# marl/l3embedding

Hardware: AMD Instinct MI355X
Metric: AVC training pairs/sec (1s audio + 224x224 frame) (higher is better)
Workload: dtype f32; 1 GPU; full cnn_L3_melspec2 AVC training step (audio+vision+fusion, fwd+bwd+Adam), batch 64 per GPU, global batch 64, fp32, inputs resident in HBM; global_batch=64, parallelism=dp1, fp32_conv=f4x4

## Files before the change

l3embedding_amd/csrc/conv_wino.hip:

```cpp
#include "kernels.h"
#include "device_common.h"
#include "wino_common.h"

#include <stdlib.h>

#include <atomic>
#include <mutex>

namespace l3 {

bool conv_wino4_selected(const ConvGeom& g);
double conv_wino4_executed_flops(const ConvGeom& g);
int conv_wino4_blocks(const ConvGeom& g, int n);
void conv_wino4_transform_weights(const float* w, float* u, const ConvGeom& g, bool from_fwd_for_dgrad, hipStream_t s);
void conv_wino4_launch(const float* x, const float* u, const float* bias, float* y, const ConvGeom& g, int n, hipStream_t s,
                       float* stat_part, int stat_mode, const BnBwdFuse* bn_bwd);

#ifdef L3_EXPERIMENTS
bool conv_wino_bx6_ok(const ConvGeom& g);
int conv_wino_bx6_blocks(const ConvGeom& g, int n);
double conv_wino_bx6_executed_flops(const ConvGeom& g);
void conv_wino_bx6_transform_weights(const float* w, float* u, const ConvGeom& g, bool from_fwd_for_dgrad, hipStream_t s);
void conv_wino_bx6_launch(const float* x, const float* u, const float* bias, float* y, const ConvGeom& g, int n, hipStream_t s,
                          float* stat_part, int stat_mode, const BnBwdFuse* bn_bwd);
#else
static inline bool conv_wino_bx6_ok(const ConvGeom&) { return false; }
static inline int conv_wino_bx6_blocks(const ConvGeom&, int) { return 0; }
static inline double conv_wino_bx6_executed_flops(const ConvGeom&) { return 0.0; }
static inline void conv_wino_bx6_transform_weights(const float*, float*, const ConvGeom&, bool, hipStream_t) {}
static inline void conv_wino_bx6_launch(const float*, const float*, const float*, float*, const ConvGeom&, int, hipStream_t, float*, int,
                                        const BnBwdFuse*) {}
#endif

namespace {

// ... 153 lines not shown
            if (c + 1 < a.nchunks) issue(0, c + 1);
            compute(1, FalseT{});
            stage_barrier();
            if (c + 1 < a.nchunks) {
                if (c + 2 < a.nchunks) issue(1, c + 2);
                compute(0, FalseT{});
                stage_barrier();
            }
        }
    };
    issue(0, 0);
    __syncthreads();
    if (xi == 1) {
        if (nu == 1) stage_loop(TrueT{}, TrueT{}); else stage_loop(TrueT{}, FalseT{});
    } else {
        if (nu == 1) stage_loop(FalseT{}, TrueT{}); else stage_loop(FalseT{}, FalseT{});
    }

    wino_output<BTX, SM, 16>(a, acc1, smem, t, wave, lane, R0, tx0, n0, mb);
    if (dyn && t == 0) {
        int nx = wq_base(0, xcd) + 8 * claim_k;
        if (nx >= total_tiles) nx = wq_claim(a.work, xcd, 1, 0, total_tiles);
        Qw[(it + 1) & 1] = nx;
    }
    }
    if (dyn && t == 0) wq_leave(a.work, (int)gridDim.x);
}

__global__ __launch_bounds__(256) void wino_weights_kernel(const float* __restrict__ w, float* __restrict__ u, int Cin,
                                                           int Cout, int dgrad) {
    const int idx = blockIdx.x * 256 + threadIdx.x;
    if (idx >= Cin * Cout) return;
    const int k = idx % Cout, c = idx / Cout;
    float g[3][3];
#pragma unroll
    for (int kh = 0; kh < 3; ++kh)
#pragma unroll
        for (int kw = 0; kw < 3; ++kw)
            g[kh][kw] = dgrad ? w[((size_t)((2 - kh) * 3 + (2 - kw)) * Cout + k) * Cin + c]
                              : w[((size_t)(kh * 3 + kw) * Cin + c) * Cout + k];
    float gg[4][3];
#pragma unroll
    for (int kw = 0; kw < 3; ++kw) {
        gg[0][kw] = g[0][kw];
        gg[1][kw] = 0.5f * (g[0][kw] + g[1][kw] + g[2][kw]);
        gg[2][kw] = 0.5f * (g[0][kw] - g[1][kw] + g[2][kw]);
        gg[3][kw] = g[2][kw];
    }
#pragma unroll
    for (int xi = 0; xi < 4; ++xi) {
        const float o0 = gg[xi][0];
        const float o1 = 0.5f * (gg[xi][0] + gg[xi][1] + gg[xi][2]);
        const float o2 = 0.5f * (gg[xi][0] - gg[xi][1] + gg[xi][2]);
        const float o3 = gg[xi][2];
        const float o[4] = {o0, o1, o2, o3};
#pragma unroll
        for (int nu = 0; nu < 4; ++nu)
            u[(((size_t)(xi * 4 + nu) * (Cin >> 2) + (c >> 2)) * Cout + k) * 4 + (c & 3)] = o[nu];
    }
}

template <int BTX, int SM>
void launch_wino2(const WinoArgs& a, hipStream_t s) {
    using G = WinoGeom<BTX>;
    static std::once_flag once[L3_MAX_DEVICES];
    int dev = 0;
    (void)hipGetDevice(&dev);
    std::call_once(once[dev & (L3_MAX_DEVICES - 1)], [] {
        (void)hipFuncSetAttribute((const void*)conv_wino_kernel<BTX, SM>, hipFuncAttributeMaxDynamicSharedMemorySize, (int)G::LDS_BYTES + 16);
    });
    static const int persist_env = l3_knob("L3_WINO_PERSIST") ? atoi(l3_knob("L3_WINO_PERSIST")) : -1;
    const int persist = persist_env >= 0 ? persist_env : 1;
    static int cus[L3_MAX_DEVICES] = {0};
    int& ncu = cus[dev & (L3_MAX_DEVICES - 1)];
    if (ncu == 0) {
        hipDeviceProp_t prop;
        ncu = hipGetDeviceProperties(&prop, dev) == hipSuccess && prop.multiProcessorCount >= 8 ? prop.multiProcessorCount / 8 * 8 : 256;
    }
    const int total = a.mblocks * a.nblocks;
    const int ncu_k = l3_knob("L3_W4_NCU") ? atoi(l3_knob("L3_W4_NCU")) / 8 * 8 : 0;
    const int ncu_eff = ncu_k > 0 && ncu_k < ncu ? ncu_k : ncu;
    const int dyn_on = l3_knob("L3_W4_DYNAMIC") ? atoi(l3_knob("L3_W4_DYNAMIC")) : a.dynamic;
    WinoArgs m = a;
    m.work = persist && total > ncu_eff && dyn_on ? persistent_work_counters(s) : nullptr;
    hipLaunchKernelGGL((conv_wino_kernel<BTX, SM>), dim3(persist && total > ncu_eff ? ncu_eff : total), dim3(1024), G::LDS_BYTES + 16, s, m);
}
template <int BTX>
void launch_wino(const WinoArgs& a, hipStream_t s) {
    if (a.stat_part != nullptr && a.bb.x != nullptr)
        launch_wino2<BTX, 2>(a, s);
    else if (a.stat_part != nullptr)
// ... 25 lines not shown
    return p;
}

}

bool conv_wino_ok(const ConvGeom& g) {
    static const int enabled = l3_knob("L3_WINOGRAD") ? atoi(l3_knob("L3_WINOGRAD")) : 1;
    return enabled && g.KH == 3 && g.KW == 3 && g.padT == 1 && g.padL == 1 && g.Ho == g.H && g.Wo == g.W &&
           g.Cin % 8 == 0 && g.Cout % 64 == 0 && (size_t)16 * g.Cin * g.Cout * 4 < (1ull << 31) &&
           (size_t)g.H * g.W * (g.Cin > g.Cout ? g.Cin : g.Cout) * 4 < (1ull << 31);
}

static int wino_chunk_samples(const ConvGeom& g) {
    const size_t per_sample = (size_t)g.H * g.W * (g.Cin > g.Cout ? g.Cin : g.Cout) * 4;
    size_t nc = ((1ull << 31) - 1) / per_sample;
    const size_t row_cap = ((1u << 22) - 1) / (size_t)((g.H + 1) / 2);
    if (nc > row_cap) nc = row_cap;
    if (nc > (size_t)g.N) nc = (size_t)g.N;
    return nc < 1 ? 1 : (int)nc;
}

static bool use_bx6(const ConvGeom& g) { return g.f2x2 == 2 && conv_wino_ok(g) && conv_wino_bx6_ok(g); }
static bool use_wino4(const ConvGeom& g) { return !use_bx6(g) && conv_wino_ok(g) && conv_wino4_selected(g); }

bool conv_wino_is_bx6(const ConvGeom& g) { return use_bx6(g); }

double conv_wino_executed_flops(const ConvGeom& g) {
    if (use_bx6(g)) return conv_wino_bx6_executed_flops(g);
    if (use_wino4(g)) return conv_wino4_executed_flops(g);
    return 2.0 * 16.0 * (double)g.N * ((g.H + 1) / 2) * ((g.W + 1) / 2) * (double)g.Cin * (double)g.Cout;
}

size_t conv_wino_floats(const ConvGeom& g) { return conv_wino_ok(g) ? (size_t)36 * g.Cin * g.Cout : 0; }

void conv_wino_transform_weights(const float* w, float* u, const ConvGeom& g, bool from_fwd_for_dgrad, hipStream_t s) {
    if (use_bx6(g)) return conv_wino_bx6_transform_weights(w, u, g, from_fwd_for_dgrad, s);
    if (use_wino4(g)) return conv_wino4_transform_weights(w, u, g, from_fwd_for_dgrad, s);
    const int total = g.Cin * g.Cout;
    hipLaunchKernelGGL(wino_weights_kernel, dim3((total + 255) / 256), dim3(256), 0, s, w, u, g.Cin, g.Cout,
                       from_fwd_for_dgrad ? 1 : 0);
}

static int stat_blocks_of(const ConvGeom& g, int algo) {
    const int nc = wino_chunk_samples(g);
    int blocks = 0;
    for (int n0 = 0; n0 < g.N; n0 += nc) {
        ConvGeom gc = g;
        gc.N = g.N - n0 < nc ? g.N - n0 : nc;
        blocks += algo == 1 ? conv_wino4_blocks(g, gc.N) : algo == 2 ? conv_wino_bx6_blocks(g, gc.N) : wino_plan(gc).mblocks;
    }
    return blocks;
}

int conv_wino_stat_blocks(const ConvGeom& g) { return conv_wino_ok(g) ? stat_blocks_of(g, use_bx6(g) ? 2 : use_wino4(g) ? 1 : 0) : 0; }

int conv_wino_stat_blocks_max(const ConvGeom& g) {
    if (!conv_wino_ok(g)) return 0;
    int m = stat_blocks_of(g, 0);
    const int b = stat_blocks_of(g, 1);
    if (b > m) m = b;
    if (g.Cin % 16 == 0 && conv_wino_bx6_ok(g)) {
        const int c = stat_blocks_of(g, 2);
        if (c > m) m = c;
    }
    return m;
}
// ... 69 lines not shown
```

l3embedding_amd/csrc/conv_wino4.hip:

```cpp
#include "kernels.h"
#include "device_common.h"

#include <stdlib.h>
#include <string.h>

#include <mutex>
#include <vector>

namespace l3 {

namespace {

struct Wino4Args {
    const float* x;
    const float* u;
    const float* bias;
    float* y;
    int N, H, W, Cin, Cout;
    int TY, TX;
    int tiles;
    int mblocks, nblocks, nchunks;
    float inv_tpi, inv_tx;
    float* stat_part;
    int stat_mode;
    BnBwdFuse bb;
    int stagger_cycles, stagger_groups;
    int lt_first, lt_end, ksplit;
    int* work;
    float* ypart;
    int solo;
    int dynamic;
    float* tail_buf;
    size_t tail_cap;
};
// ... 566 lines not shown
                        red[((jn * 2 + which) * NS + slot) * 32 + o_c32] = stv[jn][which];
                    }
                }
        }
        lds_barrier();
        if (t < 128) {
            const int c32 = t & 31, which = (t >> 5) & 1, jn = t >> 6;
            float sum = 0.f;
#pragma unroll
            for (int r = 0; r < NS; ++r) sum += red[((jn * 2 + which) * NS + r) * 32 + c32];
            a.stat_part[((size_t)mb * 2 + which) * a.Cout + n0 + jn * 32 + c32] = sum;
        }
    }
    if (!worker) __builtin_amdgcn_s_waitcnt(0x0070 | (0xF << 8));
    if (dyn && wave == 11 && lane0 == 0) {
        asm volatile("" ::: "memory");
        int nx = -1;
        if (has_next) {
            nx = wq_base(a.lt_first, xcd) + 8 * claim_k;
            if (nx >= a.lt_end) nx = wq_claim(a.work, xcd, 1, a.lt_first, a.lt_end);
        }
        Qw[it & 1] = nx;
    }
    have0 = has_next;
    }
    if (dyn && t == 0) wq_leave(a.work, (int)gridDim.x);
}

__global__ __launch_bounds__(256) void wino4_weights_kernel(const float* __restrict__ w, float* __restrict__ u, int Cin,
                                                            int Cout, int dgrad) {
    const int idx = blockIdx.x * 256 + threadIdx.x;
    if (idx >= Cin * Cout) return;
    const int k = idx % Cout, c = idx / Cout;
    float g[3][3];
#pragma unroll
    for (int kh = 0; kh < 3; ++kh)
#pragma unroll
        for (int kw = 0; kw < 3; ++kw)
            g[kh][kw] = dgrad ? w[((size_t)((2 - kh) * 3 + (2 - kw)) * Cout + k) * Cin + c]
                              : w[((size_t)(kh * 3 + kw) * Cin + c) * Cout + k];
    auto gmul = [](float a0, float a1, float a2, float* o) {
        const float s02 = a0 + a2;
        o[0] = a0;
        o[1] = (-1.f / 3.f) * (s02 + a1);
        o[2] = (1.f / 3.f) * (s02 - a1);
        o[3] = (1.f / 15.f) * fmaf(2.f, a1, fmaf(4.f, a2, a0));
        o[4] = (-4.f / 15.f) * fmaf(-2.f, a1, fmaf(4.f, a0, a2));
        o[5] = a2;
    };
    float gg[6][3];
#pragma unroll
    for (int kw = 0; kw < 3; ++kw) {
        float o[6];
        gmul(g[0][kw], g[1][kw], g[2][kw], o);
#pragma unroll
        for (int xi = 0; xi < 6; ++xi) gg[xi][kw] = o[xi];
    }
    const int c8 = c >> 3, hf = (c >> 2) & 1, sub = (c >> 1) & 1, c2 = c & 1;
#pragma unroll
    for (int xi = 0; xi < 6; ++xi) {
        float o[6];
        gmul(gg[xi][0], gg[xi][1], gg[xi][2], o);
#pragma unroll
        for (int nu = 0; nu < 6; ++nu)
            u[(((((size_t)(xi * 6 + nu) * (Cin >> 3) + c8) * 2 + sub) * 2 + hf) * Cout + k) * 2 + c2] = o[nu];
    }
}

template <int SM>
__global__ __launch_bounds__(256) void wino4_tail_reduce_kernel(Wino4Args a) {
    __shared__ float red[2][64][16];
    const int t = threadIdx.x, q = t & 3, slot = t >> 2;
    const int blk = (int)blockIdx.x >> 2, cg = (int)blockIdx.x & 3;
    const int lt = a.lt_first + blk;
    const int logical = xcd_remap(lt, a.mblocks * a.nblocks);
    const int nb = logical % a.nblocks, mb = logical / a.nblocks;
    const int n0 = nb * 64, T0 = mb * W4_TILES;
    const int cl = cg * 16 + 4 * q;
    const int ch = n0 + cl;
    f32x4 bz = {0.f, 0.f, 0.f, 0.f};
    if (a.bias != nullptr) bz = *reinterpret_cast<const f32x4*>(a.bias + ch);
    f32x4 bsc = bz, bsh = bz, bmu = bz, brs = bz;
    if constexpr (SM == 2) {
        bsc = *reinterpret_cast<const f32x4*>(a.bb.scale + ch);
        bsh = *reinterpret_cast<const f32x4*>(a.bb.shift + ch);
        bmu = *reinterpret_cast<const f32x4*>(a.bb.mean + ch);
        const f32x4 var = *reinterpret_cast<const f32x4*>(a.bb.var + ch);
#pragma unroll
        for (int c = 0; c < 4; ++c) brs[c] = rsqrtf(var[c] + a.bb.eps);
    }
    const bool srelu = SM == 1 && a.stat_mode == 2;
    float st0[4] = {0.f, 0.f, 0.f, 0.f}, st1[4] = {0.f, 0.f, 0.f, 0.f};
    const float* part = a.ypart + (size_t)blk * a.ksplit * (W4_TILES * 16 * 64) + cl;
    for (int it = 0; it < 8; ++it) {
        const int tp = it * 64 + slot, tl = tp >> 4, px = tp & 15;
        const int T = T0 + tl;
        f32x4 sum = {0.f, 0.f, 0.f, 0.f};
#pragma unroll 4
        for (int sl = 0; sl < a.ksplit; ++sl) sum += *reinterpret_cast<const f32x4*>(part + ((size_t)sl * W4_TILES * 16 + tp) * 64);
// ... 233 lines not shown
```

l3embedding_amd/csrc/engine.hip:

```cpp
#include <hip/hip_runtime.h>
#include "knobs.h"

#include <cmath>
#include <cstdio>
#include <cstdlib>
#include <cstring>
#include <map>
#include <string>
#include <vector>

#include "../../include/l3hip.h"
#include "comm.h"
#include "kernels.h"

namespace {

using namespace l3;

static thread_local std::string g_create_error;

constexpr float BN_EPS = 1e-3f;
constexpr float BN_MOMENTUM = 0.99f;
constexpr float L2_WEIGHT = 1e-5f;
constexpr float ADAM_B1 = 0.9f, ADAM_B2 = 0.999f, ADAM_EPS = 1e-8f;
// ... 8 lines not shown
    float* g = nullptr;
    int N = 0, H = 0, W = 0, C = 0;
    int64_t batch_stride = 0;
    bool alias = false;
    bool d_bf16 = false, g_bf16 = false;
    int64_t numel() const { return (int64_t)N * H * W * C; }
    int64_t rows() const { return (int64_t)N * H * W; }
};

struct Param {
    std::string name;
    int ndim = 0;
    int64_t shape[4] = {1, 1, 1, 1};
    bool trainable = false;
    int kind = 0;
    int64_t numel = 0;
    int bucket = 0;
    float* d = nullptr;
    float* g = nullptr;
};

struct Op {
    OpKind kind;
    std::string name;
    int in = 0, out = 0;
    int block = 0, bucket = 0;
    int kh = 0, kw = 0, cout = 0;
    bool same = false;
    ConvGeom geom{};
    ConvGeom dgeom{};
    int p_kernel = -1, p_bias = -1;
    float* wflip = nullptr;
    float *wino_uf = nullptr, *wino_ud = nullptr;
    int in_bn = -1;
    bool fused_first = false;
    bool defer_apply = false;
    int bn_defer = -1;
    const float* apply_coeffs = nullptr;
    float *xaug = nullptr, *gaug = nullptr;
    ConvGeom ageom{};
    int bn_follow = -1;
    int stats_nblk = 0;
    bool need_dx = true;
    int dy_to_bn = -1;
    float* xwin = nullptr;
    int bwd_part_blocks = 0;
    int p_gamma = -1, p_beta = -1, p_mmean = -1, p_mvar = -1;
    bool fused_relu = false;
    bool prerelu = false;
    int fuse_pool = -1;
    int bias_param = -1;
    bool fused_into_bn = false;
    bool bias_by_bn = false;
    float *mean = nullptr, *var = nullptr, *scale = nullptr, *shift = nullptr;
    float *biased_mean = nullptr, *biased_var = nullptr;
    PoolGeom pg{};
};

struct Tower {
    std::string prefix;
    std::vector<Tensor> t;
    std::vector<Op> ops;
    int nblocks = 0;
    int emb_conv_op = -1;
};

// ... 992 lines not shown
        }
    } else if (f.folded) {
        float* fe = e->frames;
        float* fo = e->frames + (size_t)M * f.ke;
        {
            ProfScope ps(e, F_FRONTEND, 0.0);
            frame_audio_folded(e->audio, fe, fo, B, AUDIO_T, f, e->stream);
        }
        ProfScope ps(e, F_FRONTEND, 2.0 * M * (double)f.n_dft * 2.0 * f.n_freq, nullptr,
                     2.0 * M * (double)(f.ke + f.ko) * f.nc);
        const ConvGeom ge{1, 1, M, f.ke, 1, M, f.nc, 1, 1, 0, 0}, go{1, 1, M, f.ko, 1, M, f.nc, 1, 1, 0, 0};
        conv_fwd(fe, e->wdft, nullptr, e->spec, ge, e->stream);
        conv_fwd(fo, e->wdft + (size_t)f.ke * f.nc, nullptr, e->spec + (size_t)M * f.nc, go, e->stream);
    } else {
        {
            ProfScope ps(e, F_FRONTEND, 0.0);
            frame_audio(e->audio, e->frames, B, AUDIO_T, f, e->stream);
        }
        ConvGeom g{1, 1, M, f.n_dft, 1, M, f.ncols_pad, 1, 1, 0, 0};
        ProfScope ps(e, F_FRONTEND, 2.0 * M * (double)f.n_dft * 2.0 * f.n_freq);
        conv_fwd(e->frames, e->wdft, nullptr, e->spec, g, e->stream);
    }
    {
        ProfScope ps(e, F_FRONTEND, f.n_mels ? 2.0 * B * f.n_frames * (double)f.n_freq * f.n_mels : 0.0);
        spec_to_features(e->spec, e->melw, e->mel_start, e->mel_len, e->mel_off, e->aud.t[0].d, B, f, e->stream, e->dft_nyq);
        if (f.db) db_normalize(e->aud.t[0].d, e->smax, B, e->aud.t[0].batch_stride, e->cfg.db_max_scope, e->stream);
    }
    return L3_OK;
}

static inline double act_bytes(const Tensor& t) { return (double)t.numel() * (t.d_bf16 ? 2.0 : 4.0); }
static inline double grad_bytes(const Tensor& t) { return (double)t.numel() * (t.g_bf16 ? 2.0 : 4.0); }

void tower_forward(l3_engine* e, Tower& tw, bool training) {
    for (auto& op : tw.ops) {
        Tensor& x = tw.t[op.in];
        Tensor& y = tw.t[op.out];
        switch (op.kind) {
            case OP_CONV: {
                const bool mp = e->cfg.dtype == L3_DTYPE_BF16 && conv_bf16_ok(op.geom);
                ProfScope ps(e, F_CONV_FWD, conv_flops(op.geom), op.name.c_str(),
                             op.wino_uf && !mp ? conv_wino_executed_flops(op.geom) : -1.0);
                ps.bytes(act_bytes(x) + act_bytes(y) + (double)e->params[op.p_kernel].numel * 4.0);
                static const int epi_stats = l3_knob("L3_EPILOGUE_STATS") ? atoi(l3_knob("L3_EPILOGUE_STATS")) : 1;
                if (op.wino_uf && !mp)
                    conv_wino_transform_weights(e->params[op.p_kernel].d, op.wino_uf, op.geom, false, e->stream);
                if (mp) {
                    if (x.d_bf16)
                        conv_weights_bf16(e->params[op.p_kernel].d, op.wflip, op.kh, op.kw, x.C, op.cout, true, e->stream);
                    else
                        conv_flip_weights(e->params[op.p_kernel].d, op.wflip, op.kh, op.kw, x.C, op.cout, e->stream);
                    const bool mstats = epi_stats && training && x.d_bf16 && op.bn_follow >= 0 && e->stat_scratch != nullptr;
                    conv_bf16_fwd(x.d, op.wflip, e->params[op.p_bias].d, y.d, op.geom, e->stream, x.d_bf16,
                                  mstats ? e->stat_scratch : nullptr, mstats ? (tw.ops[op.bn_follow].prerelu ? 2 : 1) : 0,
                                  y.d_bf16);
                    if (op.bn_follow >= 0) tw.ops[op.bn_follow].stats_nblk = mstats ? conv_bf16_stat_blocks(op.geom) : 0;
                    break;
                }
                if (conv_first_ok(op.geom)) {
                    const bool fstats = epi_stats && training && op.bn_follow >= 0 && e->stat_scratch != nullptr;
                    conv_first_fwd(x.d, e->params[op.p_kernel].d, e->params[op.p_bias].d, y.d, op.geom, e->stream,
                                   fstats ? e->stat_scratch : nullptr, fstats ? (tw.ops[op.bn_follow].prerelu ? 2 : 1) : 0,
                                   y.d_bf16);
                    if (op.bn_follow >= 0) tw.ops[op.bn_follow].stats_nblk = fstats ? conv_first_stat_blocks(op.geom) : 0;
                    break;
                }
                const bool stats = epi_stats && training && op.wino_uf && op.bn_follow >= 0 && e->stat_scratch != nullptr &&
                                   conv_wino_stat_blocks(op.geom) > 0;
                conv_fwd(x.d, e->params[op.p_kernel].d, e->params[op.p_bias].d, y.d, op.geom, e->stream, op.wino_uf,
                         stats ? e->stat_scratch : nullptr, stats ? (tw.ops[op.bn_follow].prerelu ? 2 : 1) : 0);
                if (op.bn_follow >= 0) tw.ops[op.bn_follow].stats_nblk = stats ? conv_wino_stat_blocks(op.geom) : 0;
                break;
            }
            case OP_BN: {
                ProfScope ps(e, F_ELEMWISE, 0.0);
                {
                    double by = !training ? 0.0 : op.stats_nblk > 0 ? (double)op.stats_nblk * 2 * x.C * 4 : act_bytes(x);
                    if (training && op.fused_first) by += act_bytes(x) + (double)x.rows() * (&op + 1)->ageom.Cin * 4.0;
                    if (op.fuse_pool >= 0) {
// ... 150 lines not shown
                    ProfScope ps(e, F_ELEMWISE, 0.0);
                    ps.bytes(grad_bytes(y));
                    colsum(y.g, e->params[op.p_bias].g, e->red_scratch, y.rows(), y.C, e->stream);
                }
                if (op.need_dx) {
                    ProfScope ps(e, F_CONV_DGRAD, conv_flops(op.geom), op.name.c_str(),
                                 op.wino_ud && !(e->cfg.dtype == L3_DTYPE_BF16 && conv_bf16_ok(op.dgeom))
                                     ? conv_wino_executed_flops(op.dgeom)
                                     : -1.0);
                    ps.bytes(grad_bytes(y) + grad_bytes(x) + (double)e->params[op.p_kernel].numel * 4.0);
                    if (!conv_dgrad_small(y.g, e->params[op.p_kernel].d, x.g, op.geom, e->stream)) {
                        if (e->cfg.dtype == L3_DTYPE_BF16 && conv_bf16_ok(op.dgeom)) {
                            if (y.g_bf16) {
                                conv_weights_bf16(e->params[op.p_kernel].d, op.wflip, op.kh, op.kw, x.C, op.cout, false,
                                                  e->stream);
                                Op* bn = training && op.dy_to_bn >= 0 && e->stat_scratch != nullptr && x.g_bf16 &&
                                                 conv_bf16_halo_ok(op.dgeom) && tw.t[tw.ops[op.dy_to_bn].in].d_bf16
                                             ? &tw.ops[op.dy_to_bn]
                                             : nullptr;
                                if (bn != nullptr && bn->fuse_pool >= 0 && (bn->xwin == nullptr || x.batch_stride != (int64_t)x.H * x.W * x.C))
                                    bn = nullptr;
                                if (bn != nullptr) {
                                    const BnBwdFuse bb{bn->fuse_pool >= 0 ? bn->xwin : tw.t[bn->in].d, bn->scale, bn->shift, bn->mean, bn->var,
                                                       BN_EPS, bn->fused_relu ? 1 : 0};
                                    conv_bf16_fwd(y.g, op.wflip, nullptr, x.g, op.dgeom, e->stream, true, e->stat_scratch, 0, true, &bb);
                                    bn->bwd_part_blocks = conv_bf16_stat_blocks(op.dgeom);
                                } else {
                                    conv_bf16_fwd(y.g, op.wflip, nullptr, x.g, op.dgeom, e->stream, true, nullptr, 0, x.g_bf16);
                                }
                            } else {
                                conv_bf16_fwd(y.g, e->params[op.p_kernel].d, nullptr, x.g, op.dgeom, e->stream);
                            }
                        } else if (op.wino_ud) {
                            conv_wino_transform_weights(e->params[op.p_kernel].d, op.wino_ud, op.dgeom, true, e->stream);
                            Op* bn = training && op.dy_to_bn >= 0 && e->stat_scratch != nullptr && !x.g_bf16 ? &tw.ops[op.dy_to_bn] : nullptr;
                            if (bn != nullptr && bn->fuse_pool >= 0 && (bn->xwin == nullptr || x.batch_stride != (int64_t)x.H * x.W * x.C))
                                bn = nullptr;
                            if (bn != nullptr && !tw.t[bn->in].d_bf16 && conv_wino_ok(op.dgeom)) {
                                const BnBwdFuse bb{bn->fuse_pool >= 0 ? bn->xwin : tw.t[bn->in].d, bn->scale, bn->shift, bn->mean, bn->var,
                                                   BN_EPS, bn->fused_relu ? 1 : 0};
                                conv_fwd(y.g, nullptr, nullptr, x.g, op.dgeom, e->stream, op.wino_ud, e->stat_scratch, 0, &bb);
                                bn->bwd_part_blocks = conv_wino_stat_blocks(op.dgeom);
                            } else {
                                conv_fwd(y.g, nullptr, nullptr, x.g, op.dgeom, e->stream, op.wino_ud);
                            }
                        } else {
                            conv_flip_weights(e->params[op.p_kernel].d, op.wflip, op.kh, op.kw, x.C, op.cout, e->stream);
                            conv_fwd(y.g, op.wflip, nullptr, x.g, op.dgeom, e->stream);
                        }
                    }
                }
                break;
            }
            default: break;
        }
    }
}

void set_solo(l3_engine* e, Tower& tw, int v) {
    for (auto& op : tw.ops)
        if (op.kind == OP_CONV) {
            op.geom.solo = op.dgeom.solo = v;
            op.geom.dynamic = op.dgeom.dynamic = e->comm != nullptr ? 1 : 0;
            float* ts = v ? e->w4_tail : nullptr;
            op.geom.tail_scratch = op.dgeom.tail_scratch = ts;
            op.geom.tail_scratch_bytes = op.dgeom.tail_scratch_bytes = ts ? conv_wino4_tail_scratch_bytes() : 0;
        }
}

void l2_sums(l3_engine* e) {
    SumsqSegs segs{};
    int nl2 = 0;
    for (auto& s : e->segments) nl2 += s.l2 ? 1 : 0;
    if (nl2 <= SUMSQ_MAX_SEGS) {
        for (auto& s : e->segments)
            if (s.l2) {
                segs.off[segs.count] = s.off;
                segs.n[segs.count++] = s.n;
            }
        sumsq_multi(e->arena_p, segs, e->l2part, e->sq_scratch, e->stream);
        return;
    }
    int si = 0;
    for (auto& s : e->segments)
        if (s.l2) sumsq(e->arena_p + s.off, s.n, e->l2part + si++, e->sq_scratch, e->stream);
}

int forward_all(l3_engine* e, bool training) {
    int rc;
    set_solo(e, e->vis, 0);
    set_solo(e, e->aud, 0);
    if (e->side && e->overlap) {
        HIPCHK(e, hipEventRecord(e->ev_fork, e->stream));
        HIPCHK(e, hipStreamWaitEvent(e->side, e->ev_fork, 0));
        l2_sums(e);
        {
            SideScope sd(e);
            if ((rc = run_frontend(e))) return rc;
            tower_forward(e, e->aud, training);
            HIPCHK(e, hipEventRecord(e->ev_join, e->stream));
        }
        tower_forward(e, e->vis, training);
        HIPCHK(e, hipStreamWaitEvent(e->stream, e->ev_join, 0));
    } else {
        l2_sums(e);
        if ((rc = run_frontend(e))) return rc;
        tower_forward(e, e->vis, training);
        tower_forward(e, e->aud, training);
    }
    ProfScope ps(e, F_HEAD, 0.0);
    const int D = e->nv + e->na;
    dense_fwd(e->h0, e->params[e->p_w1].d, e->params[e->p_b1].d, e->h1, e->B, D, e->head, 1, e->stream);
    dense_fwd(e->h1, e->params[e->p_w2].d, e->params[e->p_b2].d, e->logits, e->B, e->head, 2, 0, e->stream);
    e->last_training = training;
    return L3_OK;
}

void loss_and_head_backward(l3_engine* e, bool backward) {
    ProfScope ps(e, F_HEAD, 0.0);
    const int gb = e->cfg.global_batch > 0 ? e->cfg.global_batch : e->B;
    softmax_ce(e->logits, e->labels, e->probs, e->dlogits, e->stats, e->B, 1.0f / (float)gb, e->stream);
    if (!backward) return;
    const int D = e->nv + e->na;
    dense_bwd_w(e->h1, e->dlogits, e->params[e->p_w2].g, e->params[e->p_b2].g, e->B, e->head, 2, e->stream);
// ... 53 lines not shown
    e->bn_table = dev;
    return L3_OK;
}

int bn_stats_pack(l3_engine* e, int world) {
    int rc = ensure_bn_table(e);
    if (rc) return rc;
    if (e->bn_pack_floats == 0) return L3_OK;
    if (e->bn_send == nullptr && (rc = dev_alloc_t(e, &e->bn_send, (size_t)e->bn_pack_floats))) return rc;
    if (e->bn_gathered_world < world) {
        if ((rc = dev_alloc_t(e, &e->bn_gathered, (size_t)e->bn_pack_floats * world))) return rc;
        e->bn_gathered_world = world;
    }
    bn_moving_pack(e->bn_table, e->bn_table_n, e->bn_table_max_c, e->bn_send, e->stream);
    return L3_OK;
}

int do_update(l3_engine* e, float lr, float grad_scale) {
    {
        ProfScope ps(e, F_ADAM, 0.0);
        e->adam_t += 1;
        const double t = (double)e->adam_t;
        const float lr_t = lr * (sqrtf(1.f - powf(ADAM_B2, (float)t)) / (1.f - powf(ADAM_B1, (float)t)));
        for (size_t i = 0; i < e->segments.size(); ++i) {
            const auto& s = e->segments[i];
            int64_t n = s.n;
            const int64_t n_l2 = s.l2 ? s.n : 0;
            if (s.l2 && i + 1 < e->segments.size() && !e->segments[i + 1].l2 && e->segments[i + 1].off == s.off + s.n)
                n += e->segments[++i].n;
            adam_step(e->arena_p + s.off, e->arena_g + s.off, e->arena_m + s.off, e->arena_v + s.off, n, n_l2, 2.f * L2_WEIGHT,
                      lr_t, ADAM_B1, ADAM_B2, ADAM_EPS, grad_scale, e->stream);
        }
    }
    ProfScope ps(e, F_ELEMWISE, 0.0);
    int rc = ensure_bn_table(e);
    if (rc) return rc;
    const int replicas = e->bn_replicas_armed;
    e->bn_replicas_armed = 0;
    e->bn_step += replicas > 0 ? replicas : 1;
    bn_moving_update_all(e->bn_table, e->bn_table_n, e->bn_table_max_c, BN_MOMENTUM, e->cfg.bn_zero_debias, e->bn_step, e->stream,
                         replicas > 0 ? e->bn_gathered : nullptr, replicas, e->bn_pack_floats);
    return L3_OK;
}

int read_results(l3_engine* e, float* loss, float* acc, float* probs, float* logits) {
    HIPCHK(e, l3::stream_wait(e->stream));
    prof_collect(e);
    float st[16], l2[64];
    HIPCHK(e, hipMemcpy(st, e->stats, sizeof(st), hipMemcpyDeviceToHost));
    HIPCHK(e, hipMemcpy(l2, e->l2part, sizeof(l2), hipMemcpyDeviceToHost));
    double reg = 0.0;
    int si = 0;
    for (auto& s : e->segments)
        if (s.l2) reg += (double)L2_WEIGHT * (double)l2[si++];
    if (loss) *loss = (float)((double)st[0] / (double)e->B + reg);
    if (acc) *acc = st[1] / (float)e->B;
    if (probs) HIPCHK(e, hipMemcpy(probs, e->probs, (size_t)e->B * 2 * 4, hipMemcpyDeviceToHost));
    if (logits) HIPCHK(e, hipMemcpy(logits, e->logits, (size_t)e->B * 2 * 4, hipMemcpyDeviceToHost));
    return L3_OK;
}

int upload_inputs(l3_engine* e, const float* video, const float* audio, const float* labels) {
    const int B = e->B;
    e->staged = false;
    e->gains_valid = false;
    if (video) HIPCHK(e, hipMemcpyAsync(e->video, video, (size_t)B * 224 * 224 * 3 * 4, hipMemcpyHostToDevice, e->stream));
// ... 190 lines not shown
    if (ndim) *ndim = p.ndim;
    if (shape)
        for (int i = 0; i < 4; ++i) shape[i] = i < p.ndim ? p.shape[i] : 1;
    if (trainable) *trainable = p.trainable ? 1 : 0;
    if (numel) *numel = p.numel;
    return L3_OK;
}

static int find_param(l3_engine* e, const char* name, int64_t numel, Param** out) {
    if (!e || !name) return L3_EINVAL;
    auto it = e->pindex.find(name);
    if (it == e->pindex.end()) {
        e->err = std::string("unknown parameter: ") + name;
        return L3_EINVAL;
    }
    Param& p = e->params[it->second];
    if (p.numel != numel) {
        e->err = std::string("size mismatch for ") + name + ": expected " + std::to_string(p.numel) + " got " +
                 std::to_string(numel);
        return L3_EINVAL;
    }
    *out = &p;
    return L3_OK;
}

int l3_set_param(l3_engine* e, const char* name, const float* src, int64_t numel) {
    Param* p;
    int rc = find_param(e, name, numel, &p);
    if (rc) return rc;
    HIPCHK(e, hipSetDevice(e->cfg.device));
    HIPCHK(e, l3::stream_wait(e->stream));
    HIPCHK(e, hipMemcpy(p->d, src, (size_t)numel * 4, hipMemcpyHostToDevice));
    if (p->kind == PK_CONST) e->consts_dirty = true;
    return L3_OK;
}

int l3_get_param(l3_engine* e, const char* name, float* dst, int64_t numel) {
    Param* p;
    int rc = find_param(e, name, numel, &p);
    if (rc) return rc;
    HIPCHK(e, hipSetDevice(e->cfg.device));
    HIPCHK(e, l3::stream_wait(e->stream));
    HIPCHK(e, hipMemcpy(dst, p->d, (size_t)numel * 4, hipMemcpyDeviceToHost));
    return L3_OK;
}

int l3_get_grad(l3_engine* e, const char* name, float* dst, int64_t numel) {
    Param* p;
    int rc = find_param(e, name, numel, &p);
    if (rc) return rc;
    if (!p->trainable) {
        e->err = std::string("not trainable: ") + name;
        return L3_EINVAL;
    }
    HIPCHK(e, hipSetDevice(e->cfg.device));
    HIPCHK(e, l3::stream_wait(e->stream));
    HIPCHK(e, hipMemcpy(dst, p->g, (size_t)numel * 4, hipMemcpyDeviceToHost));
    return L3_OK;
}

int l3_reset_optimizer(l3_engine* e) {
    if (!e) return L3_EINVAL;
    HIPCHK(e, hipSetDevice(e->cfg.device));
    HIPCHK(e, hipMemsetAsync(e->arena_m, 0, (size_t)e->n_train * 4, e->stream));
    HIPCHK(e, hipMemsetAsync(e->arena_v, 0, (size_t)e->n_train * 4, e->stream));
    e->adam_t = 0;
// ... 13 lines not shown
    if (!dst || !src) return L3_EINVAL;
    if (dst == src) return L3_OK;
    if (dst->cfg.model_type != src->cfg.model_type || dst->params.size() != src->params.size() ||
        dst->n_train != src->n_train || dst->cfg.device != src->cfg.device) {
        dst->err = "l3_copy_state: engines differ in model type or device";
        return L3_EINVAL;
    }
    HIPCHK(dst, hipSetDevice(dst->cfg.device));
    HIPCHK(dst, l3::stream_wait(src->stream));
    if (src->side) HIPCHK(dst, l3::stream_wait(src->side));
    const size_t nb = (size_t)src->n_train * 4;
    HIPCHK(dst, hipMemcpyAsync(dst->arena_p, src->arena_p, nb, hipMemcpyDeviceToDevice, dst->stream));
    HIPCHK(dst, hipMemcpyAsync(dst->arena_m, src->arena_m, nb, hipMemcpyDeviceToDevice, dst->stream));
    HIPCHK(dst, hipMemcpyAsync(dst->arena_v, src->arena_v, nb, hipMemcpyDeviceToDevice, dst->stream));
    for (size_t i = 0; i < src->params.size(); ++i) {
        const Param& ps = src->params[i];
        if (ps.trainable) continue;
        HIPCHK(dst, hipMemcpyAsync(dst->params[i].d, ps.d, (size_t)ps.numel * 4, hipMemcpyDeviceToDevice, dst->stream));
    }
    Tower* dt[2] = {&dst->vis, &dst->aud};
    Tower* st[2] = {&src->vis, &src->aud};
    for (int t = 0; t < 2; ++t)
        for (size_t i = 0; i < st[t]->ops.size(); ++i) {
            const Op& so = st[t]->ops[i];
            Op& dop = dt[t]->ops[i];
            if (so.kind != OP_BN) continue;
            const size_t n = (size_t)(st[t]->t[so.in].C + 3) / 4 * 4 * 4;
            HIPCHK(dst, hipMemcpyAsync(dop.biased_mean, so.biased_mean, n, hipMemcpyDeviceToDevice, dst->stream));
            HIPCHK(dst, hipMemcpyAsync(dop.biased_var, so.biased_var, n, hipMemcpyDeviceToDevice, dst->stream));
        }
    dst->adam_t = src->adam_t;
    dst->bn_step = src->bn_step;
    dst->consts_dirty = true;
    HIPCHK(dst, l3::stream_wait(dst->stream));
    return L3_OK;
}

int l3_optimizer_steps(const l3_engine* e, int64_t* adam_t, int64_t* bn_steps) {
    if (!e) return L3_EINVAL;
    if (adam_t) *adam_t = e->adam_t;
    if (bn_steps) *bn_steps = e->bn_step;
    return L3_OK;
}

int l3_upload_batch(l3_engine* e, const float* video, const float* audio, const float* labels) {
    if (!e) return L3_EINVAL;
    HIPCHK(e, hipSetDevice(e->cfg.device));
    return upload_inputs(e, video, audio, labels);
}

int l3_upload_batch_raw(l3_engine* e, const uint8_t* video_u8, const int16_t* audio_i16, const int32_t* labels_i32) {
    if (!e) return L3_EINVAL;
    HIPCHK(e, hipSetDevice(e->cfg.device));
    const int B = e->B;
    e->staged = false;
    e->gains_valid = false;
    if (video_u8) {
        HIPCHK(e, hipMemcpyAsync(e->raw_video, video_u8, (size_t)B * 224 * 224 * 3, hipMemcpyHostToDevice, e->stream));
        preprocess_video(e->raw_video, e->video, (int64_t)B * 224 * 224 * 3, e->stream);
    }
    if (audio_i16) {
        HIPCHK(e, hipMemcpyAsync(e->raw_audio, audio_i16, (size_t)B * AUDIO_T * 2, hipMemcpyHostToDevice, e->stream));
        preprocess_audio(e->raw_audio, e->audio, (int64_t)B * AUDIO_T, e->stream);
    }
    if (labels_i32) {
        HIPCHK(e, hipMemcpyAsync(e->raw_labels, labels_i32, (size_t)B * 2 * 4, hipMemcpyHostToDevice, e->stream));
// ... 122 lines not shown
    HIPCHK(e, l3::stream_wait(e->stream));
    HIPCHK(e, hipMemcpy(gains, e->aug_gains, (size_t)e->B * sizeof(double), hipMemcpyDeviceToHost));
    return L3_OK;
}

int l3_step_forward(l3_engine* e, int training) {
    if (!e) return L3_EINVAL;
    HIPCHK(e, hipSetDevice(e->cfg.device));
    e->bucket_ready = -1;
    e->bn_replicas_armed = 0;
    e->bn_packed = false;
    if (training) {
        const int slot = (int)(e->steps_enqueued & 1);
        if (e->ev_step_set[slot]) HIPCHK(e, l3::event_wait(e->ev_step[slot]));
    }
    int rc = adopt_staged(e);
    if (rc) return rc;
    rc = forward_all(e, training != 0);
    if (rc) return rc;
    loss_and_head_backward(e, training != 0);
    e->fwd_done = true;
    HIPCHK(e, hipGetLastError());
    return L3_OK;
}

int l3_tower_step(l3_engine* e, int tower, int backward) {
    if (!e || (tower != 0 && tower != 1)) return L3_EINVAL;
    HIPCHK(e, hipSetDevice(e->cfg.device));
    int rc = adopt_staged(e);
    if (rc) return rc;
    Tower& tw = tower == 0 ? e->vis : e->aud;
    if (tower == 1 && (rc = run_frontend(e))) return rc;
    set_solo(e, tw, 1);
    tower_forward(e, tw, true);
    if (backward) {
        const int width = tower == 0 ? e->nv : e->na;
        fill(e->dh0, 1.0f / ((float)e->B * (float)width), (int64_t)e->B * (e->nv + e->na), e->stream);
        for (int b = tw.nblocks - 1; b >= 0; --b) tower_backward_block(e, tw, b, true);
    }
    e->fwd_done = false;
    HIPCHK(e, hipGetLastError());
    return L3_OK;
}

int l3_step_bucket_count(const l3_engine* e) { return e ? (int)e->buckets.size() : L3_EINVAL; }

int l3_step_backward_bucket(l3_engine* e, int bucket) {
    if (!e) return L3_EINVAL;
    if (!e->fwd_done) {
        e->err = "l3_step_backward_bucket before l3_step_forward";
        return L3_ESTATE;
    }
    if (!e->last_training && e->cfg.dtype == L3_DTYPE_BF16) {
        e->err = "inference-mode gradients are available in L3_DTYPE_F32 engines only";
        return L3_ESTATE;
    }
    HIPCHK(e, hipSetDevice(e->cfg.device));
    int rc = backward_bucket(e, bucket);
    if (rc) return rc;
    HIPCHK(e, hipGetLastError());
    return L3_OK;
}

int l3_step_update(l3_engine* e, float lr, float grad_scale) {
    if (!e) return L3_EINVAL;
    if (!e->fwd_done || !e->last_training) {
// ... 429 lines not shown
}

static int embed_rows(l3_engine* e, bool vision, const EmbedSource& src, int64_t n, int ph, int pw, int64_t D, float* out) {
    Tower& tw = vision ? e->vis : e->aud;
    const int B = e->B;
    int64_t cap_rows = (int64_t)(EMBED_OUT_BYTES / ((size_t)D * 4)) / B * B;
    if (cap_rows < B) cap_rows = B;
    const int64_t need_rows = (n + B - 1) / B * B;
    if (cap_rows > need_rows) cap_rows = need_rows;
    int rc = dev_grow_t(e, &e->emb_out, &e->emb_out_cap, (size_t)cap_rows * D);
    if (rc) return rc;
    const Tensor& t = tw.t[tw.ops[tw.emb_conv_op].out];
    PoolGeom pg{};
    pg.N = B; pg.H = t.H; pg.W = t.W; pg.C = t.C; pg.ph = ph; pg.pw = pw; pg.sh = ph; pg.sw = pw;
    tf_same(t.H, ph, ph, &pg.Ho, &pg.padT);
    tf_same(t.W, pw, pw, &pg.Wo, &pg.padL);
    pg.out_batch_stride = D;
    const size_t per = vision ? (size_t)224 * 224 * 3 : (size_t)AUDIO_T;
    float* dst_in = vision ? e->video : e->audio;
    int64_t f0 = 0;
    for (int64_t s0 = 0; s0 < n; s0 += B) {
        const int64_t cnt = n - s0 < B ? n - s0 : B;
        if (src.host) {
            HIPCHK(e, hipMemcpyAsync(dst_in, src.host + (size_t)s0 * per, (size_t)cnt * per * 4, hipMemcpyHostToDevice, e->stream));
            if (cnt < B) HIPCHK(e, hipMemsetAsync(dst_in + (size_t)cnt * per, 0, (size_t)(B - cnt) * per * 4, e->stream));
        } else {
            gather_frames(src.samples, src.table + 3 * s0, dst_in, B, (int)cnt, AUDIO_T, e->stream);
        }
        if (!vision) {
            rc = run_frontend(e);
            if (rc) return rc;
        }
        set_solo(e, tw, 1);
        tower_forward(e, tw, false);
        maxpool_fwd(t.d, e->emb_out + (size_t)(s0 - f0) * D, pg, e->stream);
        if (s0 + cnt == n || s0 + 2 * B - f0 > cap_rows) {
            HIPCHK(e, hipMemcpyAsync(out + (size_t)f0 * D, e->emb_out, (size_t)(s0 + cnt - f0) * D * 4, hipMemcpyDeviceToHost, e->stream));
            HIPCHK(e, l3::stream_wait(e->stream));
            f0 = s0 + B;
        }
    }
    prof_collect(e);
    return L3_OK;
}

static int embed_common(l3_engine* e, bool vision, const float* in, int64_t n, int ph, int pw, float* out) {
    if (!e || !in || !out || n < 0) return L3_EINVAL;
    HIPCHK(e, hipSetDevice(e->cfg.device));
    int64_t D = 0;
    int rc = embed_check(e, vision, ph, pw, &D);
    if (rc) return rc;
    EmbedSource src;
    src.host = in;
    return embed_rows(e, vision, src, n, ph, pw, D, out);
}

int l3_embed_audio(l3_engine* e, const float* audio, int64_t n, int pool_h, int pool_w, float* out) {
    return embed_common(e, false, audio, n, pool_h, pool_w, out);
}
int l3_embed_vision(l3_engine* e, const float* video, int64_t n, int pool_h, int pool_w, float* out) {
    return embed_common(e, true, video, n, pool_h, pool_w, out);
}

int l3_embed_audio_frames(l3_engine* e, const float* samples, int64_t n_samples, const int64_t* table, int64_t n_frames,
                          int pool_h, int pool_w, float* out) {
    if (!e) return L3_EINVAL;
// ... 179 lines not shown
```

l3embedding_amd/csrc/kernels.h:

```cpp
#pragma once
#include <hip/hip_runtime.h>
#include <stdint.h>

#include <string>
#include <vector>

#include "host_common.h"

namespace l3 {

struct ConvGeom {
    int N, H, W, Cin;
    int Ho, Wo, Cout;
    int KH, KW, padT, padL;
    int f2x2 = 0;
    int solo = 0;
    int dynamic = 0;
    float* tail_scratch = nullptr;
    size_t tail_scratch_bytes = 0;
};
size_t conv_wino4_tail_scratch_bytes();

struct BnBwdFuse {
    const float* x;
    const float *scale, *shift;
    const float *mean, *var;
    float eps;
    int relu;
};
void conv_fwd(const float* x, const float* w, const float* bias, float* y, const ConvGeom& g,
              hipStream_t s, const float* wino_u = nullptr, float* bn_part = nullptr, int bn_mode = 0,
              const BnBwdFuse* bn_bwd = nullptr);
bool conv_wino_ok(const ConvGeom& g);
size_t conv_wino_floats(const ConvGeom& g);
double conv_wino_executed_flops(const ConvGeom& g);
void conv_wino_transform_weights(const float* w, float* u, const ConvGeom& g, bool from_fwd_for_dgrad, hipStream_t s);
void conv_wino_fwd(const float* x, const float* u, const float* bias, float* y, const ConvGeom& g, hipStream_t s,
                   float* stat_part = nullptr, int stat_mode = 0, const BnBwdFuse* bn_bwd = nullptr);
int conv_wino_stat_blocks(const ConvGeom& g);
int conv_wino_stat_blocks_max(const ConvGeom& g);
bool conv_dgrad_small(const float* dy, const float* w, float* dx, const ConvGeom& g, hipStream_t s);
void conv_flip_weights(const float* w, float* wt, int KH, int KW, int Cin, int Cout, hipStream_t s);
size_t conv_wgrad_scratch_floats(const ConvGeom& g);
bool conv_wgrad_bf16_ok(const ConvGeom& g);
struct FirstWgFuse;
void conv_wgrad(const float* x, const float* dy, float* dw, float* part, const ConvGeom& g,
                hipStream_t s, bool bf16 = false, bool in_bf16 = false, const FirstWgFuse* first_fuse = nullptr);

bool conv_first_ok(const ConvGeom& g);
bool conv_first_wgrad_ok(const ConvGeom& g);
size_t conv_first_wgrad_scratch_floats(const ConvGeom& g);
struct FirstWgFuse {
    const void *bnx, *dA;
    const float *scale, *shift;
    const float *cA, *cB, *cC;
    int relu;
    int bf16;
};
int conv_first_wgrad(const float* x, const float* dy, float* part, const ConvGeom& g, hipStream_t s, const FirstWgFuse* fuse = nullptr);
int conv_first_stat_blocks(const ConvGeom& g);
void conv_first_fwd(const float* x, const float* w, const float* bias, void* y, const ConvGeom& g, hipStream_t s,
                    float* stat_part = nullptr, int stat_mode = 0, bool out_bf16 = false);

bool conv_wgrad_wino_ok(const ConvGeom& g);
int conv_wgrad_wino_splits(const ConvGeom& g, int n);
int conv_wgrad_wino_max_splits(const ConvGeom& g, int n);
double conv_wgrad_wino_executed_flops(const ConvGeom& g);
void conv_wgrad_wino_launch(const float* x, const float* dy, float* part, const ConvGeom& g, int n, hipStream_t s);
void conv_wgrad_wino_finish(const float* part, float* dw, const ConvGeom& g, int splits, hipStream_t s);
// ... 177 lines not shown
```

Before: 2022 pairs/s.

## Cache Winograd filter transforms and batch regeneration into one kernel after Adam

Before, every conv op re-ran its Winograd weight transform kernel inside the forward and dgrad passes. Now transformed filters are cached per op with a form tag and invalidated when weights change (after the Adam update, parameter upload, state copy). They are regenerated through a single batched kernel that handles many conv layers and writes two channels per thread with vector stores. This removes many small kernel launches from the critical path. In exchange it adds invalidation bookkeeping that must catch every weight mutation, and it does the refresh after the optimizer step instead of lazily.

```diff
diff --git a/l3embedding_amd/csrc/conv_wino.hip b/l3embedding_amd/csrc/conv_wino.hip
--- a/l3embedding_amd/csrc/conv_wino.hip
+++ b/l3embedding_amd/csrc/conv_wino.hip
@@ -1,6 +1,7 @@
 #include "kernels.h"
 #include "device_common.h"
 #include "wino_common.h"
+#include "wino_filter.h"
 
 #include <stdlib.h>
 
@@ -220,31 +221,37 @@
     const int idx = blockIdx.x * 256 + threadIdx.x;
     if (idx >= Cin * Cout) return;
     const int k = idx % Cout, c = idx / Cout;
-    float g[3][3];
-#pragma unroll
-    for (int kh = 0; kh < 3; ++kh)
-#pragma unroll
-        for (int kw = 0; kw < 3; ++kw)
-            g[kh][kw] = dgrad ? w[((size_t)((2 - kh) * 3 + (2 - kw)) * Cout + k) * Cin + c]
-                              : w[((size_t)(kh * 3 + kw) * Cin + c) * Cout + k];
-    float gg[4][3];
-#pragma unroll
-    for (int kw = 0; kw < 3; ++kw) {
-        gg[0][kw] = g[0][kw];
-        gg[1][kw] = 0.5f * (g[0][kw] + g[1][kw] + g[2][kw]);
-        gg[2][kw] = 0.5f * (g[0][kw] - g[1][kw] + g[2][kw]);
-        gg[3][kw] = g[2][kw];
-    }
-#pragma unroll
-    for (int xi = 0; xi < 4; ++xi) {
-        const float o0 = gg[xi][0];
-        const float o1 = 0.5f * (gg[xi][0] + gg[xi][1] + gg[xi][2]);
-        const float o2 = 0.5f * (gg[xi][0] - gg[xi][1] + gg[xi][2]);
-        const float o3 = gg[xi][2];
-        const float o[4] = {o0, o1, o2, o3};
-#pragma unroll
-        for (int nu = 0; nu < 4; ++nu)
-            u[(((size_t)(xi * 4 + nu) * (Cin >> 2) + (c >> 2)) * Cout + k) * 4 + (c & 3)] = o[nu];
+    float g[3][3], o[16];
+    wino_filter_taps(w, Cin, Cout, dgrad, c, k, g);
+    wino2_filter_transform(g, o);
+#pragma unroll
+    for (int pos = 0; pos < 16; ++pos) u[wino2_filter_index(pos, Cin, Cout, c, k)] = o[pos];
+}
+
+__global__ __launch_bounds__(256) void wino_filters_batched_kernel(WinoFilterBatch b) {
+    int j = 0;
+    while (j + 1 < b.count && (int)blockIdx.x >= b.first_block[j + 1]) ++j;
+    const WinoFilterJob q = b.job[j];
+    const int idx = ((int)blockIdx.x - b.first_block[j]) * 256 + threadIdx.x;
+    if (idx >= (q.Cin >> 1) * q.Cout) return;
+    const int k = idx % q.Cout, c = idx / q.Cout * 2;
+    float g0[3][3], g1[3][3];
+    wino_filter_taps(q.w, q.Cin, q.Cout, q.dgrad, c, k, g0);
+    wino_filter_taps(q.w, q.Cin, q.Cout, q.dgrad, c + 1, k, g1);
+    if (q.form == 1) {
+        float o0[36], o1[36];
+        wino4_filter_transform(g0, o0);
+        wino4_filter_transform(g1, o1);
+#pragma unroll
+        for (int pos = 0; pos < 36; ++pos)
+            *reinterpret_cast<f32x2*>(q.u + wino4_filter_index(pos, q.Cin, q.Cout, c, k)) = f32x2{o0[pos], o1[pos]};
+    } else {
+        float o0[16], o1[16];
+        wino2_filter_transform(g0, o0);
+        wino2_filter_transform(g1, o1);
+#pragma unroll
+        for (int pos = 0; pos < 16; ++pos)
+            *reinterpret_cast<f32x2*>(q.u + wino2_filter_index(pos, q.Cin, q.Cout, c, k)) = f32x2{o0[pos], o1[pos]};
     }
 }
 
@@ -336,6 +343,22 @@
 }
 
 size_t conv_wino_floats(const ConvGeom& g) { return conv_wino_ok(g) ? (size_t)36 * g.Cin * g.Cout : 0; }
+
+int conv_wino_filter_form(const ConvGeom& g) { return use_bx6(g) ? 2 : use_wino4(g) ? 1 : 0; }
+
+void conv_wino_transform_weights_batched(const WinoFilterJob* jobs, int count, hipStream_t s) {
+    for (int j0 = 0; j0 < count; j0 += WINO_FILTER_BATCH_MAX) {
+        WinoFilterBatch b{};
+        b.count = count - j0 < WINO_FILTER_BATCH_MAX ? count - j0 : WINO_FILTER_BATCH_MAX;
+        int blocks = 0;
+        for (int j = 0; j < b.count; ++j) {
+            b.job[j] = jobs[j0 + j];
+            b.first_block[j] = blocks;
+            blocks += ((b.job[j].Cin >> 1) * b.job[j].Cout + 255) / 256;
+        }
+        if (blocks > 0) hipLaunchKernelGGL(wino_filters_batched_kernel, dim3(blocks), dim3(256), 0, s, b);
+    }
+}
 
 void conv_wino_transform_weights(const float* w, float* u, const ConvGeom& g, bool from_fwd_for_dgrad, hipStream_t s) {
     if (use_bx6(g)) return conv_wino_bx6_transform_weights(w, u, g, from_fwd_for_dgrad, s);
diff --git a/l3embedding_amd/csrc/conv_wino4.hip b/l3embedding_amd/csrc/conv_wino4.hip
--- a/l3embedding_amd/csrc/conv_wino4.hip
+++ b/l3embedding_amd/csrc/conv_wino4.hip
@@ -1,5 +1,6 @@
 #include "kernels.h"
 #include "device_common.h"
+#include "wino_filter.h"
 
 #include <stdlib.h>
 #include <string.h>
@@ -632,39 +633,11 @@
     const int idx = blockIdx.x * 256 + threadIdx.x;
     if (idx >= Cin * Cout) return;
     const int k = idx % Cout, c = idx / Cout;
-    float g[3][3];
-#pragma unroll
-    for (int kh = 0; kh < 3; ++kh)
-#pragma unroll
-        for (int kw = 0; kw < 3; ++kw)
-            g[kh][kw] = dgrad ? w[((size_t)((2 - kh) * 3 + (2 - kw)) * Cout + k) * Cin + c]
-                              : w[((size_t)(kh * 3 + kw) * Cin + c) * Cout + k];
-    auto gmul = [](float a0, float a1, float a2, float* o) {
-        const float s02 = a0 + a2;
-        o[0] = a0;
-        o[1] = (-1.f / 3.f) * (s02 + a1);
-        o[2] = (1.f / 3.f) * (s02 - a1);
-        o[3] = (1.f / 15.f) * fmaf(2.f, a1, fmaf(4.f, a2, a0));
-        o[4] = (-4.f / 15.f) * fmaf(-2.f, a1, fmaf(4.f, a0, a2));
-        o[5] = a2;
-    };
-    float gg[6][3];
-#pragma unroll
-    for (int kw = 0; kw < 3; ++kw) {
-        float o[6];
-        gmul(g[0][kw], g[1][kw], g[2][kw], o);
-#pragma unroll
-        for (int xi = 0; xi < 6; ++xi) gg[xi][kw] = o[xi];
-    }
-    const int c8 = c >> 3, hf = (c >> 2) & 1, sub = (c >> 1) & 1, c2 = c & 1;
-#pragma unroll
-    for (int xi = 0; xi < 6; ++xi) {
-        float o[6];
-        gmul(gg[xi][0], gg[xi][1], gg[xi][2], o);
-#pragma unroll
-        for (int nu = 0; nu < 6; ++nu)
-            u[(((((size_t)(xi * 6 + nu) * (Cin >> 3) + c8) * 2 + sub) * 2 + hf) * Cout + k) * 2 + c2] = o[nu];
-    }
+    float g[3][3], o[36];
+    wino_filter_taps(w, Cin, Cout, dgrad, c, k, g);
+    wino4_filter_transform(g, o);
+#pragma unroll
+    for (int pos = 0; pos < 36; ++pos) u[wino4_filter_index(pos, Cin, Cout, c, k)] = o[pos];
 }
 
 template <int SM>
diff --git a/l3embedding_amd/csrc/engine.hip b/l3embedding_amd/csrc/engine.hip
--- a/l3embedding_amd/csrc/engine.hip
+++ b/l3embedding_amd/csrc/engine.hip
@@ -64,6 +64,7 @@
     int p_kernel = -1, p_bias = -1;
     float* wflip = nullptr;
     float *wino_uf = nullptr, *wino_ud = nullptr;
+    int uf_form = -1, ud_form = -1;
     int in_bn = -1;
     bool fused_first = false;
     bool defer_apply = false;
@@ -1122,6 +1123,65 @@
 static inline double act_bytes(const Tensor& t) { return (double)t.numel() * (t.d_bf16 ? 2.0 : 4.0); }
 static inline double grad_bytes(const Tensor& t) { return (double)t.numel() * (t.g_bf16 ? 2.0 : 4.0); }
 
+bool wino_cache_on() {
+    static const int on = l3_knob("L3_WINO_U_CACHE") ? atoi(l3_knob("L3_WINO_U_CACHE")) : 1;
+    return on != 0;
+}
+
+void wino_filters_stale(l3_engine* e, int p_kernel = -1) {
+    for (Tower* tw : {&e->vis, &e->aud})
+        for (auto& op : tw->ops)
+            if (op.kind == OP_CONV && (p_kernel < 0 || op.p_kernel == p_kernel)) op.uf_form = op.ud_form = -1;
+}
+
+static inline bool wino_uf_used(const l3_engine* e, const Op& op) {
+    return op.wino_uf != nullptr && !(e->cfg.dtype == L3_DTYPE_BF16 && conv_bf16_ok(op.geom));
+}
+static inline bool wino_ud_used(const l3_engine* e, const Op& op) {
+    return op.need_dx && op.wino_ud != nullptr && !(e->cfg.dtype == L3_DTYPE_BF16 && conv_bf16_ok(op.dgeom));
+}
+
+void wino_filter_ready(l3_engine* e, Op& op, bool dgrad) {
+    const ConvGeom& g = dgrad ? op.dgeom : op.geom;
+    int& have = dgrad ? op.ud_form : op.uf_form;
+    const int want = conv_wino_filter_form(g);
+    if (wino_cache_on() && have == want) return;
+    conv_wino_transform_weights(e->params[op.p_kernel].d, dgrad ? op.wino_ud : op.wino_uf, g, dgrad, e->stream);
+    have = want;
+}
+
+void wino_filters_refresh(l3_engine* e, Tower* only, bool dgrad_too) {
+    if (!wino_cache_on()) return;
+    std::vector<WinoFilterJob> jobs;
+    double bytes = 0.0;
+    std::vector<std::pair<Op*, bool>> single;
+    for (Tower* tw : {&e->vis, &e->aud}) {
+        if (only != nullptr && tw != only) continue;
+        for (auto& op : tw->ops) {
+            if (op.kind != OP_CONV) continue;
+            for (int dgrad = 0; dgrad < (dgrad_too ? 2 : 1); ++dgrad) {
+                if (!(dgrad ? wino_ud_used(e, op) : wino_uf_used(e, op))) continue;
+                const ConvGeom& g = dgrad ? op.dgeom : op.geom;
+                int& have = dgrad ? op.ud_form : op.uf_form;
+                const int want = conv_wino_filter_form(g);
+                if (have == want) continue;
+                if (want == 2 || (g.Cin & 1)) {
+                    single.push_back({&op, dgrad != 0});
+                    continue;
+                }
+                jobs.push_back(WinoFilterJob{e->params[op.p_kernel].d, dgrad ? op.wino_ud : op.wino_uf, g.Cin, g.Cout, dgrad, want});
+                bytes += (double)g.Cin * g.Cout * 4.0 * (9.0 + (want == 1 ? 36.0 : 16.0));
+                have = want;
+            }
+        }
+    }
+    if (jobs.empty() && single.empty()) return;
+    ProfScope ps(e, F_CONV_FWD, 0.0, "wino_filters");
+    ps.bytes(bytes);
+    if (!jobs.empty()) conv_wino_transform_weights_batched(jobs.data(), (int)jobs.size(), e->stream);
+    for (auto& sg : single) wino_filter_ready(e, *sg.first, sg.second);
+}
+
 void tower_forward(l3_engine* e, Tower& tw, bool training) {
     for (auto& op : tw.ops) {
         Tensor& x = tw.t[op.in];
@@ -1133,8 +1193,7 @@
                              op.wino_uf && !mp ? conv_wino_executed_flops(op.geom) : -1.0);
                 ps.bytes(act_bytes(x) + act_bytes(y) + (double)e->params[op.p_kernel].numel * 4.0);
                 static const int epi_stats = l3_knob("L3_EPILOGUE_STATS") ? atoi(l3_knob("L3_EPILOGUE_STATS")) : 1;
-                if (op.wino_uf && !mp)
-                    conv_wino_transform_weights(e->params[op.p_kernel].d, op.wino_uf, op.geom, false, e->stream);
+                if (op.wino_uf && !mp) wino_filter_ready(e, op, false);
                 if (mp) {
                     if (x.d_bf16)
                         conv_weights_bf16(e->params[op.p_kernel].d, op.wflip, op.kh, op.kw, x.C, op.cout, true, e->stream);
@@ -1351,7 +1410,7 @@
                                 conv_bf16_fwd(y.g, e->params[op.p_kernel].d, nullptr, x.g, op.dgeom, e->stream);
                             }
                         } else if (op.wino_ud) {
-                            conv_wino_transform_weights(e->params[op.p_kernel].d, op.wino_ud, op.dgeom, true, e->stream);
+                            wino_filter_ready(e, op, true);
                             Op* bn = training && op.dy_to_bn >= 0 && e->stat_scratch != nullptr && !x.g_bf16 ? &tw.ops[op.dy_to_bn] : nullptr;
                             if (bn != nullptr && bn->fuse_pool >= 0 && (bn->xwin == nullptr || x.batch_stride != (int64_t)x.H * x.W * x.C))
                                 bn = nullptr;
@@ -1409,6 +1468,7 @@
     int rc;
     set_solo(e, e->vis, 0);
     set_solo(e, e->aud, 0);
+    wino_filters_refresh(e, nullptr, training);
     if (e->side && e->overlap) {
         HIPCHK(e, hipEventRecord(e->ev_fork, e->stream));
         HIPCHK(e, hipStreamWaitEvent(e->side, e->ev_fork, 0));
@@ -1528,6 +1588,8 @@
                       lr_t, ADAM_B1, ADAM_B2, ADAM_EPS, grad_scale, e->stream);
         }
     }
+    wino_filters_stale(e);
+    wino_filters_refresh(e, nullptr, true);
     ProfScope ps(e, F_ELEMWISE, 0.0);
     int rc = ensure_bn_table(e);
     if (rc) return rc;
@@ -1784,6 +1846,7 @@
     HIPCHK(e, l3::stream_wait(e->stream));
     HIPCHK(e, hipMemcpy(p->d, src, (size_t)numel * 4, hipMemcpyHostToDevice));
     if (p->kind == PK_CONST) e->consts_dirty = true;
+    if (p->kind == PK_KERNEL) wino_filters_stale(e, (int)(p - e->params.data()));
     return L3_OK;
 }
 
@@ -1863,6 +1926,7 @@
     dst->adam_t = src->adam_t;
     dst->bn_step = src->bn_step;
     dst->consts_dirty = true;
+    wino_filters_stale(dst);
     HIPCHK(dst, l3::stream_wait(dst->stream));
     return L3_OK;
 }
@@ -2051,6 +2115,7 @@
     Tower& tw = tower == 0 ? e->vis : e->aud;
     if (tower == 1 && (rc = run_frontend(e))) return rc;
     set_solo(e, tw, 1);
+    wino_filters_refresh(e, &tw, backward != 0);
     tower_forward(e, tw, true);
     if (backward) {
         const int width = tower == 0 ? e->nv : e->na;
@@ -2546,6 +2611,7 @@
             if (rc) return rc;
         }
         set_solo(e, tw, 1);
+        wino_filters_refresh(e, &tw, false);
         tower_forward(e, tw, false);
         maxpool_fwd(t.d, e->emb_out + (size_t)(s0 - f0) * D, pg, e->stream);
         if (s0 + cnt == n || s0 + 2 * B - f0 > cap_rows) {
diff --git a/l3embedding_amd/csrc/kernels.h b/l3embedding_amd/csrc/kernels.h
--- a/l3embedding_amd/csrc/kernels.h
+++ b/l3embedding_amd/csrc/kernels.h
@@ -35,6 +35,20 @@
 size_t conv_wino_floats(const ConvGeom& g);
 double conv_wino_executed_flops(const ConvGeom& g);
 void conv_wino_transform_weights(const float* w, float* u, const ConvGeom& g, bool from_fwd_for_dgrad, hipStream_t s);
+int conv_wino_filter_form(const ConvGeom& g);
+struct WinoFilterJob {
+    const float* w;
+    float* u;
+    int Cin, Cout;
+    int dgrad, form;
+};
+constexpr int WINO_FILTER_BATCH_MAX = 32;
+struct WinoFilterBatch {
+    WinoFilterJob job[WINO_FILTER_BATCH_MAX];
+    int first_block[WINO_FILTER_BATCH_MAX];
+    int count;
+};
+void conv_wino_transform_weights_batched(const WinoFilterJob* jobs, int count, hipStream_t s);
 void conv_wino_fwd(const float* x, const float* u, const float* bias, float* y, const ConvGeom& g, hipStream_t s,
                    float* stat_part = nullptr, int stat_mode = 0, const BnBwdFuse* bn_bwd = nullptr);
 int conv_wino_stat_blocks(const ConvGeom& g);
diff --git a/l3embedding_amd/csrc/wino_filter.h b/l3embedding_amd/csrc/wino_filter.h
--- /dev/null
+++ b/l3embedding_amd/csrc/wino_filter.h
@@ -0,0 +1,63 @@
+#pragma once
+#include <hip/hip_runtime.h>
+
+namespace l3 {
+
+__device__ __forceinline__ void wino_filter_taps(const float* __restrict__ w, int Cin, int Cout, int dgrad, int c, int k,
+                                                 float (&g)[3][3]) {
+#pragma unroll
+    for (int kh = 0; kh < 3; ++kh)
+#pragma unroll
+        for (int kw = 0; kw < 3; ++kw)
+            g[kh][kw] = dgrad ? w[((size_t)((2 - kh) * 3 + (2 - kw)) * Cout + k) * Cin + c]
+                              : w[((size_t)(kh * 3 + kw) * Cin + c) * Cout + k];
+}
+
+__device__ __forceinline__ void wino2_filter_transform(const float (&g)[3][3], float (&o)[16]) {
+    float gg[4][3];
+#pragma unroll
+    for (int kw = 0; kw < 3; ++kw) {
+        gg[0][kw] = g[0][kw];
+        gg[1][kw] = 0.5f * (g[0][kw] + g[1][kw] + g[2][kw]);
+        gg[2][kw] = 0.5f * (g[0][kw] - g[1][kw] + g[2][kw]);
+        gg[3][kw] = g[2][kw];
+    }
+#pragma unroll
+    for (int xi = 0; xi < 4; ++xi) {
+        o[xi * 4 + 0] = gg[xi][0];
+        o[xi * 4 + 1] = 0.5f * (gg[xi][0] + gg[xi][1] + gg[xi][2]);
+        o[xi * 4 + 2] = 0.5f * (gg[xi][0] - gg[xi][1] + gg[xi][2]);
+        o[xi * 4 + 3] = gg[xi][2];
+    }
+}
+__device__ __forceinline__ size_t wino2_filter_index(int pos, int Cin, int Cout, int c, int k) {
+    return (((size_t)pos * (Cin >> 2) + (c >> 2)) * Cout + k) * 4 + (c & 3);
+}
+
+__device__ __forceinline__ void wino4_filter_gmul(float a0, float a1, float a2, float* o) {
+    const float s02 = a0 + a2;
+    o[0] = a0;
+    o[1] = (-1.f / 3.f) * (s02 + a1);
+    o[2] = (1.f / 3.f) * (s02 - a1);
+    o[3] = (1.f / 15.f) * fmaf(2.f, a1, fmaf(4.f, a2, a0));
+    o[4] = (-4.f / 15.f) * fmaf(-2.f, a1, fmaf(4.f, a0, a2));
+    o[5] = a2;
+}
+__device__ __forceinline__ void wino4_filter_transform(const float (&g)[3][3], float (&o)[36]) {
+    float gg[6][3];
+#pragma unroll
+    for (int kw = 0; kw < 3; ++kw) {
+        float t[6];
+        wino4_filter_gmul(g[0][kw], g[1][kw], g[2][kw], t);
+#pragma unroll
+        for (int xi = 0; xi < 6; ++xi) gg[xi][kw] = t[xi];
+    }
+#pragma unroll
+    for (int xi = 0; xi < 6; ++xi) wino4_filter_gmul(gg[xi][0], gg[xi][1], gg[xi][2], o + xi * 6);
+}
+__device__ __forceinline__ size_t wino4_filter_index(int pos, int Cin, int Cout, int c, int k) {
+    const int c8 = c >> 3, hf = (c >> 2) & 1, sub = (c >> 1) & 1, c2 = c & 1;
+    return (((((size_t)pos * (Cin >> 3) + c8) * 2 + sub) * 2 + hf) * Cout + k) * 2 + c2;
+}
+
+}
```

Result: no change. 2017 pairs/s (-0.2%).
